# ilia-glushchenko/SimplePathTracer

Hardware: AMD Instinct MI355X
Metric: Msamples/s (pixels×spp/s), RTIOW random-sphere scene, 1/2/4/8 MI355X (higher is better)
Workload: dtype f32

## Files before the change

### simplepathtracer_amd/csrc/spt_device.h

```cpp
#pragma once
#include <hip/hip_runtime.h>
#include <stdint.h>

#include "spt_powf.h"

#pragma clang fp contract(off)

namespace spt {

constexpr uint32_t SPT_SKYBOX_ID = 0, SPT_REFLECTIVE_ID = 1, SPT_REFRACTIVE_ID = 2, SPT_DIFFUSE_ID = 3;

struct f3 {
    float x, y, z;
};

__device__ __forceinline__ f3 mk(float x, float y, float z) { return f3{x, y, z}; }
__device__ __forceinline__ f3 add(f3 a, f3 b) { return f3{a.x + b.x, a.y + b.y, a.z + b.z}; }
__device__ __forceinline__ f3 sub(f3 a, f3 b) { return f3{a.x - b.x, a.y - b.y, a.z - b.z}; }
__device__ __forceinline__ f3 mul(f3 a, float s) { return f3{a.x * s, a.y * s, a.z * s}; }
__device__ __forceinline__ f3 neg(f3 a) { return f3{-a.x, -a.y, -a.z}; }
__device__ __forceinline__ float dot(f3 a, f3 b) { return (a.x * b.x + a.y * b.y) + a.z * b.z; }
__device__ __forceinline__ float lensq(f3 a) { return (a.x * a.x + a.y * a.y) + a.z * a.z; }
__device__ __forceinline__ float sqrt_pos_normal(float h)
{
    float s = __builtin_amdgcn_sqrtf(h);
    const float dn = __builtin_bit_cast(float, __builtin_bit_cast(int, s) - 1);
    const float up = __builtin_bit_cast(float, __builtin_bit_cast(int, s) + 1);
    const float rdn = __builtin_fmaf(-dn, s, h);
    const float rup = __builtin_fmaf(-up, s, h);
    s = rdn <= 0.0f ? dn : s;
    s = rup > 0.0f ? up : s;
    return s;
}

struct Recip {
    float b, rc;
};
__device__ __forceinline__ Recip recip(float b)
{
    float rc = __builtin_amdgcn_rcpf(b);
    const float e = __builtin_fmaf(-b, rc, 1.0f);
    rc = __builtin_fmaf(e, rc, rc);
    return Recip{b, rc};
}
__device__ __forceinline__ float div_core(float a, Recip r)
{
    float q = a * r.rc;
    float e = __builtin_fmaf(-r.b, q, a);
    q = __builtin_fmaf(e, r.rc, q);
    e = __builtin_fmaf(-r.b, q, a);
    return __builtin_fmaf(e, r.rc, q);
}
__device__ __forceinline__ bool div_operand_ok(float x)
{
    const float ax = __builtin_fabsf(x);
    return ax >= 0x1p-40f && ax <= 0x1p40f;
}
__device__ __forceinline__ float div_rn(float a, float b)
{
    float q = div_core(a, recip(b));
    if (__builtin_expect(!(div_operand_ok(a) && div_operand_ok(b)), 0)) q = a / b;
    return q;
}

__device__ __forceinline__ f3 normalize(f3 a)
{
    const float L = lensq(a);
    const Recip r = recip(sqrt_pos_normal(L));
    f3 out = f3{div_core(a.x, r), div_core(a.y, r), div_core(a.z, r)};
    if (__builtin_expect(!(div_operand_ok(a.x) && div_operand_ok(a.y) && div_operand_ok(a.z)), 0)) {
        const float l = __builtin_sqrtf(L);
        out = f3{a.x / l, a.y / l, a.z / l};
    }
    return out;
}
__device__ __forceinline__ f3 reflect(f3 v, f3 n) { return sub(v, mul(mul(n, dot(v, n)), 2.0f)); }

constexpr uint64_t kGamma = 0x9E3779B97F4A7C15ull;

__device__ __forceinline__ uint64_t fmix64(uint64_t z)
{
    z = (z ^ (z >> 30)) * 0xBF58476D1CE4E5B9ull;
    z = (z ^ (z >> 27)) * 0x94D049BB133111EBull;
    return z ^ (z >> 31);
}

__device__ __forceinline__ uint32_t next_u32(uint64_t &st)
{
    st += kGamma;
    uint64_t z = st;
    z = (z ^ (z >> 30)) * 0xBF58476D1CE4E5B9ull;
    z = (z ^ (z >> 27)) * 0x94D049BB133111EBull;
    return (uint32_t)((z ^ (z >> 31)) >> 31);
}

__device__ __forceinline__ float canon_u32(uint32_t bits)
{
    float u = (float)bits * 2.3283064365386963e-10f;
    return u >= 1.0f ? 0x1.fffffep-1f : u;
}
__device__ __forceinline__ float uniform_bits(uint32_t bits, float a, float b)
{
    const float f = __builtin_fminf((float)bits, 0x1.fffffep+31f);
    return __builtin_fmaf(f, 0x1p-32f * (b - a), a);
}
__device__ __forceinline__ float uniform(uint64_t &st, float a, float b) { return uniform_bits(next_u32(st), a, b); }


__device__ __forceinline__ float pow5f(float x) { return spt_glibc_powf(x, 5.f); }

__device__ __forceinline__ float schlick(float rsq, float c) { return rsq + (1.f - rsq) * pow5f(1.f - c); }

__device__ __forceinline__ float refract_k(float r, float c) { return r * c - __builtin_sqrtf(1.f - r * r * (1.f - c * c)); }
__device__ __forceinline__ f3 refract_dir(f3 d, f3 n, float r, float c)
{
    return normalize(add(mul(d, r), mul(n, refract_k(r, c))));
}

__device__ __forceinline__ bool no_tir(float r, float c) { return r * __builtin_sqrtf(1.f - c * c) < 1.f; }

__device__ __forceinline__ uint8_t f2u8(float v)
{
    if (!(v > -2147483648.0f && v < 2147483648.0f)) return 0;
    return (uint8_t)(int32_t)v;
}
__device__ __forceinline__ uint8_t gamma_byte(float c)
{
    return f2u8(__builtin_roundf(__builtin_sqrtf(c / 255.f) * 255.f));
}

}
```

### simplepathtracer_amd/csrc/spt_internal.h

```cpp
#pragma once
#include <hip/hip_runtime.h>
#include <stdint.h>

#include "spt_hip.h"
#include "spt_codes.h"

namespace spt {

struct RowMap {
    uint32_t y0, y1, strip, parts, part;
    uint32_t x0, width;
};

__host__ __device__ inline uint32_t row_of(const RowMap &m, uint32_t lr)
{
    uint32_t blk = lr / m.strip;
    return m.y0 + (blk * m.parts + m.part) * m.strip + (lr - blk * m.strip);
}

__host__ __device__ inline uint32_t rows_owned(const RowMap &m)
{
    if (m.y1 <= m.y0) return 0;
    uint32_t h = m.y1 - m.y0;
    uint32_t period = m.strip * m.parts;
    uint32_t full = h / period, rem = h % period;
    uint32_t r = full * m.strip;
    uint32_t start = m.part * m.strip;
    if (rem > start) r += (rem - start < m.strip) ? rem - start : m.strip;
    return r;
}

__host__ __device__ inline void tile_pixel(uint32_t q, uint32_t width, uint32_t rows, uint32_t &lr, uint32_t &col)
{
    const uint32_t band = (q / width) >> 3;
    const uint32_t h = rows - (band << 3) < 8u ? rows - (band << 3) : 8u;
    const uint32_t qb = q - band * 8u * width;
    const uint32_t ft = width >> 3, wr = width & 7u;
    uint32_t row, c;
    if (h == 8u) {
        const uint32_t t = qb >> 6;
        if (t < ft) {
            row = (qb >> 3) & 7u;
            c = (t << 3) | (qb & 7u);
        } else {
            const uint32_t e = qb - (ft << 6);
            row = e / wr;
            c = (ft << 3) + (e - row * wr);
        }
    } else {
        const uint32_t th = h << 3;
        const uint32_t t = qb / th;
        if (t < ft) {
            const uint32_t e = qb - t * th;
            row = e >> 3;
            c = (t << 3) | (e & 7u);
        } else {
            const uint32_t e = qb - ft * th;
            row = e / wr;
            c = (ft << 3) + (e - row * wr);
        }
    }
    lr = (band << 3) + row;
    col = c;
}


__host__ __device__ inline uint32_t row_of_fast(const RowMap &m, uint32_t lr, const FastDiv &div_strip)
{
    const uint32_t blk = fast_div(lr, div_strip);
    return m.y0 + (blk * m.parts + m.part) * m.strip + (lr - blk * m.strip);
}

struct DealRule {
    uint64_t below;
    uint32_t q, rem;
};
constexpr DealRule make_deal_rule(uint32_t np)
{
    DealRule r{0ull, 0u, 0u};
    if (np == 0u || np > 64u) return r;
    r.q = 64u / np;
    r.rem = 64u - r.q * np;
    uint32_t start = 0;
    for (uint32_t k = 0; k < np; ++k) {
        if (start > 0u) r.below |= 1ull << (start - 1u);
        start += r.q + (k < r.rem ? 1u : 0u);
    }
    return r;
}
struct DealTable {
    DealRule e[65];
    constexpr DealTable() : e{}
    {
        for (uint32_t np = 0; np <= 64u; ++np) e[np] = make_deal_rule(np);
    }
};
static constexpr DealTable kDealTable{};
__host__ __device__ inline uint32_t deal_start(const DealRule &r, uint32_t rank)
{
    return rank * r.q + (rank < r.rem ? rank : r.rem);
}
__host__ __device__ inline uint32_t deal_count(const DealRule &r, uint32_t rank)
{
    return r.q + (rank < r.rem ? 1u : 0u);
}
__host__ __device__ inline void deal_lane(const DealRule &r, uint32_t lane, uint32_t &rank, uint32_t &tt)
{
#ifdef __HIP_DEVICE_COMPILE__
    rank = __builtin_amdgcn_mbcnt_hi((uint32_t)(r.below >> 32), __builtin_amdgcn_mbcnt_lo((uint32_t)r.below, 0u));
#else
    rank = (uint32_t)__builtin_popcountll(r.below & ((1ull << lane) - 1ull));
#endif
    tt = lane - deal_start(r, rank);
}

__host__ __device__ inline void ts_item(uint32_t q, uint32_t width, uint32_t rows, uint32_t S, const FastDiv &div_band,
                                        const FastDiv &div_tile, uint32_t &sl, uint32_t &lr, uint32_t &col)
{
    const uint32_t band = rows >= 8u ? fast_div(q, div_band) : 0u;
    const uint32_t h = rows - (band << 3) < 8u ? rows - (band << 3) : 8u;
    const uint32_t qb = q - band * 8u * width * S;
    const uint32_t ft = width >> 3, wr = width & 7u;
    const uint32_t ti = h * 8u * S;
    uint32_t e, wt, c0;
    if (h == 8u) {
        const uint32_t t = fast_div(qb, div_tile);
        if (t < ft) {
            e = qb - t * 64u * S;
            sl = e >> 6;
            const uint32_t pix = e & 63u;
            lr = (band << 3) + (pix >> 3);
            col = (t << 3) + (pix & 7u);
            return;
        }
        e = qb - ft * ti;
        wt = wr;
        c0 = ft << 3;
    } else {
        const uint32_t t = qb / ti;
        wt = t < ft ? 8u : wr;
        e = qb - (t < ft ? t : ft) * ti;
        c0 = (t < ft ? t : ft) << 3;
    }
    sl = e / (h * wt);
    const uint32_t pix = e - sl * h * wt;
    const uint32_t row = pix / wt;
    lr = (band << 3) + row;
    col = c0 + (pix - row * wt);
}

__host__ __device__ inline void ts_slot_base(uint32_t lr, uint32_t col, uint32_t width, uint32_t rows, uint32_t S,
                                             uint32_t &q0, uint32_t &step)
{
    const uint32_t band = lr >> 3;
    const uint32_t h = rows - (band << 3) < 8u ? rows - (band << 3) : 8u;
    const uint32_t ft = width >> 3, wr = width & 7u;
    const uint32_t t = col >> 3;
    const uint32_t tc = t < ft ? t : ft;
    const uint32_t wt = t < ft ? 8u : wr;
    q0 = band * 8u * width * S + tc * h * 8u * S + (lr - (band << 3)) * wt + (col - (tc << 3));
    step = h * wt;
}


constexpr uint32_t kMaxGroup = 16;
constexpr uint32_t kClusterSlots = 8;
constexpr uint32_t kFlatLeafSlots = 4;
constexpr double kFlatScale = 1.0 - 1e-4;
constexpr double kBoxS = 1.63e-3;
constexpr float kBoxMinDir = 0x1p-20f;
constexpr uint32_t kNoSlot = 0xFFFFFFFFu;
constexpr uint32_t kMiss = 0xFFFFFFFFu;

struct AccelView {
    const float4 *slots;
    const uint32_t *orig;
    const void *nodes;
    uint32_t always_groups, n_nodes;
    uint32_t tree;
    uint32_t leaf_slots;
    const float *kpre;
    float pre_cm;
};

struct PrimLists {
    const uint2 *b8, *b4;
    const uint32_t *slots;
    uint32_t bw;
    uint32_t on;
};
constexpr uint32_t kPrimWalk = 0xFFFFFFFFu;

struct DeviceScene {
    const float4 *shade;
    const uint32_t *mat;
    uint32_t n;
    uint32_t code_stride, code_jmax;
    AccelView accel;
};

struct Camera {
    float view[12];
    float eye[3];
    float sky[3];
};

struct BatchRect {
    uint32_t item_off, item_end, slot_off, pix_off;
    uint32_t x0, y0, w, rows;
    uint32_t npix, alias;
    uint8_t *rgb8;
    FastDiv div_band, div_tile;
};
static_assert(sizeof(BatchRect) == 72, "BatchRect layout");
constexpr uint32_t kInlineRects = 4;

struct RenderArgs {
    DeviceScene scene;
    Camera cam;
    uint32_t width, height, bounces, mode;
    uint64_t seed_key;
    RowMap map;
    uint32_t npix;
    uint32_t spp_batch;
    uint32_t s0;
    uint32_t n_items;
    uint32_t claim;
    FastDiv div_band, div_tile;
    FastDiv div_strip;
    uint32_t *samples;
    uint32_t slot_words;
    uint32_t *head;
    unsigned long long *counters;
    const BatchRect *rects;
    uint32_t n_rects;
    uint32_t n_queues, queue_items;
    uint32_t inline_rects;
    BatchRect rects_inline[kInlineRects];
    uint32_t *svc_ctl;
    const struct SvcJob *svc_jobs;
    const uint32_t *svc_job_claim;
    uint32_t *svc_done;
    unsigned long long *svc_trace;
    uint32_t *svc_host;
    const struct SvcJob *svc_host_jobs;
    const uint32_t *svc_host_job_claim;
    PrimLists prim;
};

constexpr uint32_t kMaxQueues = 8, kQueueStride = 64;
// ... 198 lines not shown
```

### simplepathtracer_amd/csrc/spt_path.h

```cpp
#pragma once
#include "spt_device.h"
#include "spt_internal.h"

#include <float.h>

#ifndef SPT_GROUP
#define SPT_GROUP 4
#endif

#ifndef SPT_DIAG
#define SPT_DIAG 0
#endif
#ifndef SPT_LEAF_SPLIT
#define SPT_LEAF_SPLIT 1
#endif
#ifndef SPT_DUP
#define SPT_DUP 0
#endif
#ifndef SPT_SAMPLER_SKIP0
#define SPT_SAMPLER_SKIP0 1
#endif
#ifndef SPT_SAMPLER_EVEN
#define SPT_SAMPLER_EVEN 1
#endif
// ... 637 lines not shown
    const float ds = lensq(sub(o, p));
    bool better = front && ds < h.best;
    if (__builtin_expect(front && ds == h.best && h.idx != kMiss, 0)) better = orig[s] < orig[h.idx];
    h.best = better ? ds : h.best;
    h.idx = better ? s : h.idx;
    h.t = better ? t : h.t;
}

#ifndef SPT_LANE_LEAF_T
#define SPT_LANE_LEAF_T 24
#endif
#ifndef SPT_LANE_GROUP
#define SPT_LANE_GROUP 2
#endif
#ifndef SPT_LANE_STEPS
#define SPT_LANE_STEPS 8
#endif
template <int LEAF, bool BYTES = false>
__device__ __forceinline__ bool lane_cast(const AccelView &ac, const f3 &o, const f3 &d, bool active, CastDiag &dg,
                                          const uint32_t *lnodes, bool fresh, uint32_t budget, Hit &h, uint32_t &i,
                                          uint32_t &leaf, uint32_t &leaf2)
{
    if (fresh) {
        h.idx = kMiss;
        h.best = FLT_MAX;
        h.t = 0.f;
        i = active ? 0u : (BYTES ? ac.n_nodes << 5 : ac.n_nodes);
        leaf = leaf2 = kNoSlot;
    }
    const float dod = dot(o, d);
    cfloat *slots = (cfloat *)ac.slots;
    const float ddev = lensq(d) - 1.0f;
    const bool no_cull = active && !(ddev <= 1e-6f && ddev >= -1e-6f);
    const float oo = lensq(o);
    if (SPT_DIAG) dg.live_now = (uint32_t)__popcll(__ballot(active));
    for (uint32_t g = 0; g < ac.always_groups; ++g) {
        float4 g4[SPT_GROUP];
#pragma unroll
        for (int k = 0; k < SPT_GROUP; ++k) g4[k] = ld_uniform(slots, g * SPT_GROUP + k);
        test_group<SPT_GROUP>(g4, ac.orig, g * SPT_GROUP, o, d, dod, h, dg);
    }
    auto rcp_dir = [](float x) {
        const float m = __builtin_fmaxf(__builtin_fabsf(x), kBoxMinDir);
        return __builtin_amdgcn_rcpf(__builtin_copysignf(m, x));
    };
    const bool nocull = no_cull || (active && !(oo <= 1e30f));
    float irx, iry, irz, qlx, qly, qlz, qhx, qhy, qhz, neta, kn, sbl;
    auto near_bound = [&](float best) { return __builtin_fmaf(__builtin_amdgcn_sqrtf(best), 1.00001f, kn); };
    auto walk_terms = [&]() {
        const float olen = __builtin_amdgcn_sqrtf(lensq(o)) * 1.000001f;
        const float el = __builtin_fmaf((float)kBoxS, olen, 1e-6f);
        irx = rcp_dir(d.x);
        iry = rcp_dir(d.y);
        irz = rcp_dir(d.z);
        qlx = (-o.x - el) * irx;
        qly = (-o.y - el) * iry;
        qlz = (-o.z - el) * irz;
        qhx = (el - o.x) * irx;
        qhy = (el - o.y) * iry;
        qhz = (el - o.z) * irz;
        const float obs = olen + ac.pre_cm;
        neta = -__builtin_fmaf(1e-6f, obs, 1e-6f);
        kn = __builtin_fmaf(1e-5f, obs, 1e-6f);
        sbl = near_bound(h.best);
    };
    walk_terms();
    const uint4 *ln = (const uint4 *)lnodes;
    const float4 *__restrict__ gs = ac.slots;
    const uint32_t n = BYTES ? ac.n_nodes << 5 : ac.n_nodes;
    uint32_t it = 0;
    for (;;) {
        if (++it > budget) break;
        const bool tr = i < n && leaf2 == kNoSlot;
        const unsigned long long mt = __ballot(tr);
        const unsigned long long mp = __ballot(leaf != kNoSlot);
        if ((mt | mp) == 0ull) break;
        if (mp != 0ull && (mt == 0ull || __popcll(mp) >= SPT_LANE_LEAF_T)) {
            if (SPT_DIAG) {
                const unsigned long long nl = (unsigned long long)__popcll(mp);
                dg.leaves += 1;
                dg.pairs += nl;
                dg.lane_tests += (unsigned long long)LEAF * nl;
            }
            if (leaf != kNoSlot) {
#pragma unroll 1
                for (int k0 = 0; k0 < LEAF; k0 += SPT_LANE_GROUP) {
                    float4 m[SPT_LANE_GROUP];
#pragma unroll
                    for (int k = 0; k < SPT_LANE_GROUP; ++k) m[k] = gs[leaf + k0 + k];
#pragma unroll
                    for (int k = 0; k < SPT_LANE_GROUP; ++k) {
                        float tc, hh;
                        if (ray_sphere(m[k], o, d, tc, hh))
                            update_member_lane(tc, hh, ac.orig, leaf + k0 + k, o, d, dod, h);
                    }
                }
                sbl = near_bound(h.best);
                leaf = leaf2;
                leaf2 = kNoSlot;
            }
            continue;
        }
        if (SPT_DIAG) dg.live += 1;
        auto visit = [&]() {
            const uint4 *rec = BYTES ? (const uint4 *)((const char *)lnodes + i) : ln + 2 * i;
            const uint4 ra = rec[0], rb = rec[1];
            const uint32_t nskip = rb.x, nslot = rb.y;
            const float ax = __builtin_fmaf(__uint_as_float(ra.x), irx, qlx);
            const float bx = __builtin_fmaf(__uint_as_float(ra.w), irx, qhx);
            const float ay = __builtin_fmaf(__uint_as_float(ra.y), iry, qly);
            const float by = __builtin_fmaf(__uint_as_float(rb.z), iry, qhy);
            const float az = __builtin_fmaf(__uint_as_float(ra.z), irz, qlz);
            const float bz = __builtin_fmaf(__uint_as_float(rb.w), irz, qhz);
            const float tn = max3_raw(__builtin_fminf(ax, bx), __builtin_fminf(ay, by),
                                      max_raw(__builtin_fminf(az, bz), neta));
            const float tf = min3_raw(__builtin_fmaxf(ax, bx), __builtin_fmaxf(ay, by),
                                      min_raw(__builtin_fmaxf(az, bz), sbl));
            const bool hit = (tn <= tf) | nocull;
            const bool is_leaf = nslot != kNoSlot;
            if (hit && is_leaf) {
                leaf2 = leaf;
                leaf = nslot;
            }
            i = (hit && !is_leaf) ? i + (BYTES ? 32u : 1u) : nskip;
        };
#pragma unroll
        for (int k = 0; k < SPT_LANE_STEPS; ++k) {
            const bool w = i < n && leaf2 == kNoSlot;
            if (SPT_DIAG) dg.nodes += (unsigned long long)__popcll(__ballot(w));
            if (w) visit();
        }
    }
    return !(i < n || leaf != kNoSlot);
}

template <int LEAF>
__device__ __forceinline__ Hit find_closest_lane(const AccelView &ac, const f3 &o, const f3 &d, bool active,
                                                 CastDiag &dg, const uint32_t *lnodes)
{
    Hit h;
    uint32_t i, leaf, leaf2;
    (void)lane_cast<LEAF>(ac, o, d, active, dg, lnodes, true, 0xFFFFFFFFu, h, i, leaf, leaf2);
    return h;
}

struct Path {
    uint32_t phase, item, bounce, spec;
    uint64_t st;
    f3 o, d;
    uint32_t slot;
    uint32_t job;
};

__device__ __forceinline__ f3 coop_ball_vector(uint64_t &st, bool need, uint32_t *lds, unsigned long long *rounds = nullptr)
{
    const uint32_t lane = __lane_id();
    const uint64_t st0 = st;
    f3 r;
    uint32_t jacc = 0;
    unsigned long long pend;
    uint32_t jb;
    const unsigned long long needm = __ballot(need);
    if (SPT_SAMPLER_SKIP0 && __popcll(needm) <= 32) {
        r = mk(0.f, 0.f, 0.f);
        pend = needm;
        jb = 0;
    } else {
        uint64_t t = st0;
        r.x = uniform(t, -0.5f, 0.5f);
        r.y = uniform(t, -0.5f, 0.5f);
        r.z = uniform(t, -0.5f, 0.5f);
        pend = __ballot(need && lensq(r) < 0.25f);
        jb = 1;
    }
    const uint32_t s_lo = (uint32_t)st0, s_hi = (uint32_t)(st0 >> 32);
    if (SPT_DIAG && rounds) rounds[0] += 1;
#if SPT_DIAG
    const unsigned long long t_in = __builtin_amdgcn_s_memtime();
#endif
#if SPT_SAMPLER_EVEN
    if (jb != 0u) jacc = __builtin_amdgcn_inverse_ballot_w64(pend) ? 1u : 0u;
    while (pend != 0ull) {
        if (SPT_DIAG && rounds) rounds[1] += 1;
        const DealRule dr = kDealTable.e[__popcll(pend)];
        const bool is_p = __builtin_amdgcn_inverse_ballot_w64(pend);
        const uint32_t rank = lane_rank(pend);
        if (is_p) lds[rank] = (jacc << 6) | lane;
        uint32_t pidx, tt;
        deal_lane(dr, lane, pidx, tt);
        const uint32_t w = lds[pidx];
        const uint32_t src = w & 63u;
        const uint32_t h_lo = (uint32_t)__shfl((int)s_lo, (int)src), h_hi = (uint32_t)__shfl((int)s_hi, (int)src);
        uint64_t b = (((uint64_t)h_hi << 32) | h_lo) + (uint64_t)(3u * ((w >> 6) + tt)) * kGamma;
        f3 c;
        c.x = uniform(b, -0.5f, 0.5f);
        c.y = uniform(b, -0.5f, 0.5f);
        c.z = uniform(b, -0.5f, 0.5f);
        const unsigned long long acc = __ballot(!(lensq(c) < 0.25f));
        const uint32_t start = deal_start(dr, rank), cnt = deal_count(dr, rank);
        const unsigned long long seg = acc >> (start & 63u);
        const uint32_t tstar = seg != 0ull ? (uint32_t)__builtin_ctzll(seg) : 64u;
        const bool found = is_p && tstar < cnt;
        const uint32_t from = found ? start + tstar : lane;
        const float rx = __shfl(c.x, (int)from), ry = __shfl(c.y, (int)from), rz = __shfl(c.z, (int)from);
        if (found) r = mk(rx, ry, rz);
        if (is_p) jacc += tstar < cnt ? tstar : cnt;
        pend = __ballot(is_p && !found);
    }
#else
    while (pend != 0ull) {
        if (SPT_DIAG && rounds) rounds[1] += 1;
        const uint32_t np = (uint32_t)__popcll(pend);
        uint32_t lg = np <= 4u ? 4u : (uint32_t)__builtin_clz(np - 1u) - 26u;
        lg = lg > 4u ? 4u : lg;
        const bool is_p = __builtin_amdgcn_inverse_ballot_w64(pend);
        const uint32_t rank = lane_rank(pend);
        if (is_p) lds[rank] = lane;
        const uint32_t pidx = lane >> lg, tt = lane & ((1u << lg) - 1u);
        const bool valid = pidx < np;
        const uint32_t src = lds[valid ? pidx : 0u];
        const uint32_t h_lo = (uint32_t)__shfl((int)s_lo, (int)src), h_hi = (uint32_t)__shfl((int)s_hi, (int)src);
        uint64_t b = (((uint64_t)h_hi << 32) | h_lo) + (uint64_t)(3u * (jb + tt)) * kGamma;
        f3 c;
        c.x = uniform(b, -0.5f, 0.5f);
        c.y = uniform(b, -0.5f, 0.5f);
        c.z = uniform(b, -0.5f, 0.5f);
        const unsigned long long acc = __ballot(valid && !(lensq(c) < 0.25f));
        const uint32_t seg = is_p ? (uint32_t)(acc >> (rank << lg)) & ((1u << (1u << lg)) - 1u) : 0u;
        const bool found = seg != 0u;
        const uint32_t tstar = found ? (uint32_t)__builtin_ctz(seg) : 0u;
        const uint32_t from = found ? (rank << lg) + tstar : lane;
        const float rx = __shfl(c.x, (int)from), ry = __shfl(c.y, (int)from), rz = __shfl(c.z, (int)from);
        if (found) {
            r = mk(rx, ry, rz);
            jacc = jb + tstar;
        }
        pend = __ballot(is_p && !found);
        jb += 1u << lg;
    }
#endif
    if (need) st = st0 + (uint64_t)(3u * (jacc + 1u)) * kGamma;
#if SPT_DIAG
    if (rounds) rounds[2] += __builtin_amdgcn_s_memtime() - t_in;
#endif
    return r;
}

typedef __attribute__((address_space(4))) const RenderArgs kargs_t;
__device__ __forceinline__ kargs_t *kernarg_args()
{
    uint32_t z;
    asm volatile("s_mov_b32 %0, 0" : "=s"(z));
    typedef __attribute__((address_space(4))) const char kchar;
    return (kargs_t *)((kchar *)__builtin_amdgcn_kernarg_segment_ptr() + z);
}

__device__ __forceinline__ bool prim_list_cast(const AccelView &ac, const f3 &o, const f3 &d, bool active, uint32_t pxy,
                                               Hit &h, CastDiag &dg)
{
    kargs_t &k = *kernarg_args();
    const float ddev = lensq(d) - 1.0f;
    if (__ballot(active && !(ddev <= 1e-6f && ddev >= -1e-6f && lensq(o) <= 1e30f)) != 0ull) return false;
    h.idx = kMiss;
    h.best = FLT_MAX;
    h.t = 0.f;
    const unsigned long long live = __ballot(active);
    if (live == 0ull) return true;
    const uint32_t bw = k.prim.bw;
    const uint32_t x = pxy & 0xFFFFu, y = pxy >> 16;
    const float dod = dot(o, d);
    cfloat *slots = (cfloat *)ac.slots;
    cuint *ids = (cuint *)k.prim.slots;
    if (SPT_DIAG) dg.live_now = (uint32_t)__popcll(live);
    auto test_run = [&](uint2 e) {
        for (uint32_t i = e.x; i < e.x + e.y; i += 4u) {
            uint32_t s[4];
            float4 sp[4];
#pragma unroll
            for (int q = 0; q < 4; ++q) s[q] = ids[i + q];
#pragma unroll
            for (int q = 0; q < 4; ++q) sp[q] = ld_uniform(slots, s[q]);
            float tcv[4], hv[4];
            bool pass[4];
#pragma unroll
            for (int q = 0; q < 4; ++q) pass[q] = ray_sphere(sp[q], o, d, tcv[q], hv[q]);
            if (SPT_DIAG) dg.lane_tests += 4ull * dg.live_now;
#pragma unroll
            for (int q = 0; q < 4; ++q) {
                const unsigned long long pm = __ballot(pass[q]);
                if (SPT_DIAG) {
                    dg.spheres += 1;
                    dg.branches += pm != 0ull ? 1 : 0;
                }
                if (pm != 0ull) update_member(pm, tcv[q], hv[q], ac.orig, s[q], o, d, dod, h, dg);
            }
        }
    };
    const uint32_t b8 = (y >> 3) * bw + (x >> 3);
    const uint32_t lead = __builtin_amdgcn_readlane(b8, (int)__builtin_ctzll(live));
    if (__ballot(active && b8 != lead) == 0ull) {
        cuint *blk = (cuint *)k.prim.b8 + 2u * lead;
        const uint2 e = make_uint2(blk[0], blk[1]);
        if (e.y == kPrimWalk) return false;
        test_run(e);
        return true;
    }
    const uint32_t b4 = (y >> 2) * bw + (x >> 3);
    unsigned long long todo = live;
    while (todo != 0ull) {
        const uint32_t b = __builtin_amdgcn_readlane(b4, (int)__builtin_ctzll(todo));
        cuint *blk = (cuint *)k.prim.b4 + 2u * b;
        const uint2 e = make_uint2(blk[0], blk[1]);
        if (e.y == kPrimWalk) return false;
        test_run(e);
        todo &= ~__ballot(active && b4 == b);
    }
    return true;
}

__device__ __forceinline__ void refract_event(const float4 *__restrict__ slots, Path &ps, uint32_t idx)
{
    const float4 cs = slots[idx];
    const f3 C = mk(cs.x, cs.y, cs.z);
    const f3 nrm = normalize(sub(ps.o, C));
    const f3 d = ps.d;
    const float cc = dot(neg(nrm), d);
    f3 nd;
    if (uniform(ps.st, 0.f, 1.f) < schlick(kRsq, cc)) {
        nd = reflect(d, nrm);
    } else if (no_tir(kAirToGlass, cc)) {
        const f3 d2 = refract_dir(d, nrm, kAirToGlass, cc);
        const f3 rs = sub(C, ps.o);
        const float tc = dot(rs, d2);
        const float dd = lensq(rs) - tc * tc;
        const float t = tc + __builtin_sqrtf(cs.w - dd);
        ps.o = mk(ps.o.x + d2.x * t, ps.o.y + d2.y * t, ps.o.z + d2.z * t);
        const f3 n2 = neg(normalize(sub(ps.o, C)));
        const float c2 = dot(neg(n2), d2);
        if (uniform(ps.st, 0.f, 1.f) < schlick(kRsq, c2))
            nd = reflect(d2, n2);
        else if (no_tir(kGlassToAir, c2))
            nd = refract_dir(d2, n2, kGlassToAir, c2);
        else
            nd = reflect(d2, n2);
    } else {
        nd = reflect(d, nrm);
    }
    ps.d = nd;
}

template <bool WT = false>
__device__ __forceinline__ void finish_step(uint32_t mode, uint32_t *samples, Path &ps, bool fin, bool spec_event,
                                            bool refr_event, bool sky, uint32_t word, unsigned long long &done,
                                            unsigned long long &dropped)
{
    bool counted = true;
    if (spec_event) {
        const uint32_t k = ps.spec & 0xFFFFu;
        if (mode == 1u && k < kTaskPasses && refr_event) ps.spec |= 1u << (16u + k);
        ++ps.spec;
        if (mode == 1u && k + 1u >= kTaskPasses) {
            fin = true;
            counted = false;
            word = kZeroWord;
            ++dropped;
        } else if (k + 1u > kSpecularCap) {
            fin = true;
            word = kZeroWord;
        }
    }
    if (fin) {
        typedef __attribute__((address_space(1))) uint32_t gu32_t;
        typedef __attribute__((address_space(1))) unsigned long long gu64_t;
        if (mode == 0u) {
            if (WT)
                __hip_atomic_store((gu32_t *)(samples + ps.item), word, __ATOMIC_RELAXED, __HIP_MEMORY_SCOPE_AGENT);
            else
                samples[ps.item] = word;
        } else {
            const uint32_t key =
                counted ? 1u + (((ps.spec & 0xFFFFu) << 11) | (sky ? 1u << 10 : 0u) | ((ps.spec >> 16) & 0x3FFu)) : 0u;
            if (WT)
                __hip_atomic_store((gu64_t *)(samples + (size_t)2 * ps.item), (unsigned long long)word | ((unsigned long long)key << 32),
                                   __ATOMIC_RELAXED, __HIP_MEMORY_SCOPE_AGENT);
            else
                *(uint2 *)(samples + (size_t)2 * ps.item) = make_uint2(word, key);
        }
        ps.phase = PH_IDLE;
        ps.d = mk(0.f, 0.f, 0.f);
        ++done;
    }
}

template <bool KARG, bool WT, bool SAMPLER>
__device__ __forceinline__ void shade_step_body(const RenderArgs &a, Path &ps, const Hit &h, bool act,
                                                unsigned long long &done, unsigned long long &dropped, uint32_t *lds,
                                                unsigned long long *diag_rounds)
{
    const float4 *__restrict__ hit = a.scene.accel.slots;
    const float4 *__restrict__ shade = a.scene.shade;
    const uint32_t *__restrict__ mat = a.scene.mat;
    uint32_t *samples = a.samples;
    uint32_t mode = a.mode;
    uint32_t bounces = a.bounces, code_stride = a.scene.code_stride, code_jmax = a.scene.code_jmax;
    if constexpr (KARG) {
        kargs_t &k = *kernarg_args();
        hit = k.scene.accel.slots;
        shade = k.scene.shade;
        mat = k.scene.mat;
        samples = k.samples;
        mode = k.mode;
        bounces = k.bounces;
        code_stride = k.scene.code_stride;
        code_jmax = k.scene.code_jmax;
    }
    const uint32_t idx = h.idx;
    bool fin = false;
    uint32_t word = kZeroWord;
    const bool dl = ps.phase == PH_DLOOP;
    uint32_t m = SPT_SKYBOX_ID;
    if (act && idx != kMiss) m = mat[idx];
    bool scatter = false, refr = false;
    if (!act) {
    } else if (dl) {
        --ps.bounce;
        const bool end = ps.bounce == 0u || idx == kMiss;
        if (end) {
            const uint32_t j = min(bounces - ps.bounce - 1u, code_jmax);
            word = code_word(diffuse_code(j, ps.slot, code_stride));
            fin = true;
        }
        scatter = !end;
        refr = false;
    } else {
        scatter = m == SPT_DIFFUSE_ID || m == SPT_REFLECTIVE_ID;
        refr = m == SPT_REFRACTIVE_ID;
        if (!scatter && !refr) {
            word = __float_as_uint(ps.d.y + 1.f);
            fin = true;
        }
    }
    bool spec_event = false;
    const f3 rv_coop = SAMPLER ? coop_ball_vector(ps.st, scatter, lds, diag_rounds) : opaque_v3(mk(0.1f, 0.2f, 0.3f));
    if ((SPT_DUP & 2) && SAMPLER) {
        uint64_t st2 = opaque_v(ps.st);
        const f3 r2 = coop_ball_vector(st2, opaque_v(scatter ? 1u : 0u) != 0u, lds);
        sink_v(r2.x);
        sink_v(r2.y);
        sink_v(r2.z);
        sink_v(st2);
    }
    if (scatter) {
        const float4 cs = hit[idx];
        const f3 C = mk(cs.x, cs.y, cs.z);
        ps.o = contact(ps.o, ps.d, h.t);
        const f3 nrm = normalize(sub(ps.o, C));
        f3 rv = rv_coop;
        f3 base;
        if (dl) {
            base = add(ps.o, nrm);
        } else if (m == SPT_DIFFUSE_ID) {
            ps.slot = idx;
            base = nrm;
            ps.phase = PH_DLOOP;
        } else {
            base = reflect(ps.d, nrm);
            rv = mul(rv, shade[idx].w);
            spec_event = true;
        }
        ps.d = normalize(add(base, rv));
    }
    if (refr) {
        ps.o = contact(ps.o, ps.d, h.t);
        if (SPT_DUP & 256) {
            Path p2 = ps;
            p2.o = opaque_v3(p2.o);
            refract_event(hit, p2, idx);
            sink_v(p2.d.x);
            sink_v(p2.o.x);
            sink_v(p2.st);
        }
        refract_event(hit, ps, idx);
        spec_event = true;
    }
    finish_step<WT>(mode, samples, ps, fin, spec_event, refr, !dl, word, done, dropped);
}
template <bool KARG = false, bool WT = false>
__device__ __forceinline__ void shade_step(const RenderArgs &a, Path &ps, const Hit &h, bool act,
                                           unsigned long long &done, unsigned long long &dropped, uint32_t *lds,
                                           unsigned long long *diag_rounds = nullptr)
{
    if (SPT_DUP & 128) {
        Path p2 = ps;
        p2.o = opaque_v3(p2.o);
        p2.d = opaque_v3(p2.d);
        Hit h2 = h;
        h2.t = opaque_v(h2.t);
        unsigned long long d2 = 0, x2 = 0;
        shade_step_body<KARG, WT, false>(a, p2, h2, act, d2, x2, lds, nullptr);
        sink_v(p2.o.x);
        sink_v(p2.d.x);
        sink_v(p2.st);
    }
    shade_step_body<KARG, WT, true>(a, ps, h, act, done, dropped, lds, diag_rounds);
}



__device__ __forceinline__ void start_path(const RenderArgs &a, uint32_t mine, uint32_t rows, const Recip &rw,
                                           const Recip &rh, const f3 &eye, Path &ps, uint32_t *pxy = nullptr)
{
    uint32_t sl, lr, cx;
    ts_item(mine, a.map.width, rows, a.spp_batch, a.div_band, a.div_tile, sl, lr, cx);
    const uint32_t s = a.s0 + sl;
    ps.item = mine;
    const uint32_t x = a.map.x0 + cx;
    const uint32_t y = a.map.parts == 1u ? a.map.y0 + lr : row_of_fast(a.map, lr, a.div_strip);
    if (pxy) *pxy = (y << 16) | x;
    ps.st = fmix64(a.seed_key ^ (((uint64_t)(y * a.width + x) << 32) | (uint64_t)s));
    const float un = (float)y + uniform(ps.st, -1.f, 1.f);
    const float vn = (float)x + uniform(ps.st, -1.f, 1.f);
    float u = div_core(un, rw), v = div_core(vn, rh);
    if (__builtin_expect(!(div_operand_ok(un) && div_operand_ok(vn)), 0)) {
        u = un / (float)a.width;
        v = vn / (float)a.height;
    }
    const float vx = -1.f + 2.f * v, vy = -1.f + 2.f * u;
    const float *m = a.cam.view;
    ps.d = normalize(mk((m[0] * vx + m[1] * vy) + (m[2] * 1.f + m[3] * 0.f),
                        (m[4] * vx + m[5] * vy) + (m[6] * 1.f + m[7] * 0.f),
                        (m[8] * vx + m[9] * vy) + (m[10] * 1.f + m[11] * 0.f)));
    ps.o = eye;
    ps.phase = PH_TRACE;
    ps.bounce = a.bounces;
    ps.spec = 0;
}

__device__ __forceinline__ void start_path_kernarg(uint32_t mine, uint32_t rows, Path &ps, uint32_t *pxy = nullptr)
{
    kargs_t &k = *kernarg_args();
    RenderArgs a;
    a.map = RowMap{k.map.y0, k.map.y1, k.map.strip, k.map.parts, k.map.part, k.map.x0, k.map.width};
    a.width = k.width;
    a.height = k.height;
    a.bounces = k.bounces;
    a.npix = k.npix;
    a.n_items = k.n_items;
    a.spp_batch = k.spp_batch;
    a.s0 = k.s0;
    a.seed_key = k.seed_key;
    a.div_band = FastDiv{k.div_band.d, k.div_band.m, k.div_band.s};
    a.div_tile = FastDiv{k.div_tile.d, k.div_tile.m, k.div_tile.s};
    a.div_strip = FastDiv{k.div_strip.d, k.div_strip.m, k.div_strip.s};
#pragma unroll
    for (int q = 0; q < 12; ++q) a.cam.view[q] = k.cam.view[q];
    start_path(a, mine, rows, recip((float)a.width), recip((float)a.height),
               mk(k.cam.eye[0], k.cam.eye[1], k.cam.eye[2]), ps, pxy);
}

typedef __attribute__((address_space(4))) const BatchRect crect_t;
__device__ __forceinline__ uint32_t find_rect(uint32_t nb)
{
    kargs_t &k = *kernarg_args();
    crect_t *r = k.inline_rects ? (crect_t *)k.rects_inline : (crect_t *)k.rects;
    uint32_t lo = 0, hi = k.n_rects;
    while (hi - lo > 1u) {
        const uint32_t mid = (lo + hi) >> 1;
        if (r[mid].item_off <= nb) lo = mid; else hi = mid;
    }
    return lo;
}

__device__ __forceinline__ void start_path_rect(uint32_t mine, uint32_t ri, Path &ps, uint32_t *pxy = nullptr)
{
    kargs_t &k = *kernarg_args();
    crect_t &r = (k.inline_rects ? (crect_t *)k.rects_inline : (crect_t *)k.rects)[ri];
    if (mine >= r.item_end) return;
    RenderArgs a;
    a.map = RowMap{r.y0, r.y0 + r.rows, 1u, 1u, 0u, r.x0, r.w};
    a.width = k.width;
    a.height = k.height;
    a.bounces = k.bounces;
    a.npix = r.npix;
    a.spp_batch = k.spp_batch;
    a.s0 = k.s0;
    a.seed_key = k.seed_key;
    a.div_band = FastDiv{r.div_band.d, r.div_band.m, r.div_band.s};
    a.div_tile = FastDiv{r.div_tile.d, r.div_tile.m, r.div_tile.s};
    a.div_strip = FastDiv{1u, 0u, 0u};
#pragma unroll
    for (int q = 0; q < 12; ++q) a.cam.view[q] = k.cam.view[q];
    start_path(a, mine - r.item_off, r.rows, recip((float)a.width), recip((float)a.height),
               mk(k.cam.eye[0], k.cam.eye[1], k.cam.eye[2]), ps, pxy);
    ps.item += r.slot_off;
}

__device__ __forceinline__ void start_path_svc(uint32_t mine, const uint32_t *rec, Path &ps, uint32_t *pxy = nullptr)
{
    auto f = [&](int i) -> uint32_t { return (uint32_t)__builtin_amdgcn_readfirstlane(rec[i]); };
    if (mine >= f(1)) return;
    kargs_t &k = *kernarg_args();
    RenderArgs a;
    a.map = RowMap{f(8), f(9), f(10), f(11), f(12), f(13), f(14)};
    a.width = k.width;
    a.height = k.height;
    a.bounces = k.bounces;
    a.spp_batch = f(5);
    a.s0 = f(6);
    a.seed_key = k.seed_key;
    a.div_band = FastDiv{f(15), f(16), f(17)};
    a.div_tile = FastDiv{f(18), f(19), f(20)};
    a.div_strip = FastDiv{f(21), f(22), f(23)};
#pragma unroll
    for (int q = 0; q < 12; ++q) a.cam.view[q] = k.cam.view[q];
    start_path(a, mine - f(0), f(4), recip((float)a.width), recip((float)a.height),
               mk(k.cam.eye[0], k.cam.eye[1], k.cam.eye[2]), ps, pxy);
    ps.item += f(2);
    ps.job = f(3);
}

}
}
```

Baseline: 25710.

## Convert shade step control flow to wave-uniform ballot masks

Rewrites the shading step so material classification, termination and scatter decisions are held as 64-bit wave ballot masks (SGPRs) rather than per-lane booleans. Lane predicates are recovered with inverse_ballot, and normalize's slow-path check uses min3/max3 plus a ballot. The sampler loads its deal table as 16-byte scalar loads from constant memory, and finish_step gets a specialized early path for mode 0. The aim is to cut VALU compare and exec-mask bookkeeping and divergent branching in the hot shading loop, at the cost of inline asm and heavier reliance on compiler handling of the ballot intrinsics.

```diff
diff --git a/simplepathtracer_amd/csrc/spt_device.h b/simplepathtracer_amd/csrc/spt_device.h
--- a/simplepathtracer_amd/csrc/spt_device.h
+++ b/simplepathtracer_amd/csrc/spt_device.h
@@ -63,14 +63,25 @@
     return q;
 }
 
+__device__ __forceinline__ unsigned long long normalize_slow_mask(f3 a, float L)
+{
+    float lo, hi;
+    asm("v_min3_f32 %0, |%1|, |%2|, |%3|" : "=v"(lo) : "v"(a.x), "v"(a.y), "v"(a.z));
+    asm("v_max3_f32 %0, |%1|, |%2|, |%3|" : "=v"(hi) : "v"(a.x), "v"(a.y), "v"(a.z));
+    return __ballot(!(lo >= 0x1p-40f)) | __ballot(!(hi <= 0x1p40f)) | __ballot(!(L <= 0x1p82f));
+}
 __device__ __forceinline__ f3 normalize(f3 a)
 {
     const float L = lensq(a);
     const Recip r = recip(sqrt_pos_normal(L));
     f3 out = f3{div_core(a.x, r), div_core(a.y, r), div_core(a.z, r)};
-    if (__builtin_expect(!(div_operand_ok(a.x) && div_operand_ok(a.y) && div_operand_ok(a.z)), 0)) {
+    const unsigned long long slow = normalize_slow_mask(a, L);
+    if (__builtin_expect(slow != 0ull, 0)) {
+        const bool mine = __builtin_amdgcn_inverse_ballot_w64(slow);
         const float l = __builtin_sqrtf(L);
-        out = f3{a.x / l, a.y / l, a.z / l};
+        out.x = mine ? a.x / l : out.x;
+        out.y = mine ? a.y / l : out.y;
+        out.z = mine ? a.z / l : out.z;
     }
     return out;
 }
diff --git a/simplepathtracer_amd/csrc/spt_internal.h b/simplepathtracer_amd/csrc/spt_internal.h
--- a/simplepathtracer_amd/csrc/spt_internal.h
+++ b/simplepathtracer_amd/csrc/spt_internal.h
@@ -95,7 +95,7 @@
         for (uint32_t np = 0; np <= 64u; ++np) e[np] = make_deal_rule(np);
     }
 };
-static constexpr DealTable kDealTable{};
+alignas(16) static constexpr DealTable kDealTable{};
 __host__ __device__ inline uint32_t deal_start(const DealRule &r, uint32_t rank)
 {
     return rank * r.q + (rank < r.rem ? rank : r.rem);
diff --git a/simplepathtracer_amd/csrc/spt_path.h b/simplepathtracer_amd/csrc/spt_path.h
--- a/simplepathtracer_amd/csrc/spt_path.h
+++ b/simplepathtracer_amd/csrc/spt_path.h
@@ -813,7 +813,7 @@
     uint32_t job;
 };
 
-__device__ __forceinline__ f3 coop_ball_vector(uint64_t &st, bool need, uint32_t *lds, unsigned long long *rounds = nullptr)
+__device__ __forceinline__ f3 coop_ball_vector(uint64_t &st, unsigned long long needm, uint32_t *lds, unsigned long long *rounds = nullptr)
 {
     const uint32_t lane = __lane_id();
     const uint64_t st0 = st;
@@ -821,7 +821,6 @@
     uint32_t jacc = 0;
     unsigned long long pend;
     uint32_t jb;
-    const unsigned long long needm = __ballot(need);
     if (SPT_SAMPLER_SKIP0 && __popcll(needm) <= 32) {
         r = mk(0.f, 0.f, 0.f);
         pend = needm;
@@ -831,7 +830,7 @@
         r.x = uniform(t, -0.5f, 0.5f);
         r.y = uniform(t, -0.5f, 0.5f);
         r.z = uniform(t, -0.5f, 0.5f);
-        pend = __ballot(need && lensq(r) < 0.25f);
+        pend = needm & __ballot(lensq(r) < 0.25f);
         jb = 1;
     }
     const uint32_t s_lo = (uint32_t)st0, s_hi = (uint32_t)(st0 >> 32);
@@ -841,9 +840,14 @@
 #endif
 #if SPT_SAMPLER_EVEN
     if (jb != 0u) jacc = __builtin_amdgcn_inverse_ballot_w64(pend) ? 1u : 0u;
+    typedef uint32_t u32x4 __attribute__((ext_vector_type(4)));
+    typedef __attribute__((address_space(4))) const u32x4 cu32x4;
+    cu32x4 *deal = (cu32x4 *)&kDealTable.e[0];
+    asm volatile("" : "+s"(deal));
     while (pend != 0ull) {
         if (SPT_DIAG && rounds) rounds[1] += 1;
-        const DealRule dr = kDealTable.e[__popcll(pend)];
+        const u32x4 dw = deal[__popcll(pend)];
+        const DealRule dr{((uint64_t)dw.y << 32) | dw.x, dw.z, dw.w};
         const bool is_p = __builtin_amdgcn_inverse_ballot_w64(pend);
         const uint32_t rank = lane_rank(pend);
         if (is_p) lds[rank] = (jacc << 6) | lane;
@@ -861,12 +865,13 @@
         const uint32_t start = deal_start(dr, rank), cnt = deal_count(dr, rank);
         const unsigned long long seg = acc >> (start & 63u);
         const uint32_t tstar = seg != 0ull ? (uint32_t)__builtin_ctzll(seg) : 64u;
-        const bool found = is_p && tstar < cnt;
+        const unsigned long long foundm = pend & __ballot(tstar < cnt);
+        const bool found = __builtin_amdgcn_inverse_ballot_w64(foundm);
         const uint32_t from = found ? start + tstar : lane;
         const float rx = __shfl(c.x, (int)from), ry = __shfl(c.y, (int)from), rz = __shfl(c.z, (int)from);
         if (found) r = mk(rx, ry, rz);
         if (is_p) jacc += tstar < cnt ? tstar : cnt;
-        pend = __ballot(is_p && !found);
+        pend &= ~foundm;
     }
 #else
     while (pend != 0ull) {
@@ -900,7 +905,7 @@
         jb += 1u << lg;
     }
 #endif
-    if (need) st = st0 + (uint64_t)(3u * (jacc + 1u)) * kGamma;
+    if (__builtin_amdgcn_inverse_ballot_w64(needm)) st = st0 + (uint64_t)(3u * (jacc + 1u)) * kGamma;
 #if SPT_DIAG
     if (rounds) rounds[2] += __builtin_amdgcn_s_memtime() - t_in;
 #endif
@@ -1011,13 +1016,33 @@
 }
 
 template <bool WT = false>
-__device__ __forceinline__ void finish_step(uint32_t mode, uint32_t *samples, Path &ps, bool fin, bool spec_event,
-                                            bool refr_event, bool sky, uint32_t word, unsigned long long &done,
-                                            unsigned long long &dropped)
-{
+__device__ __forceinline__ void finish_step(uint32_t mode, uint32_t *samples, Path &ps, unsigned long long finm,
+                                            unsigned long long specm, unsigned long long refrm, unsigned long long skym,
+                                            uint32_t word, unsigned long long &done, unsigned long long &dropped)
+{
+    typedef __attribute__((address_space(1))) uint32_t gu32_t;
+    typedef __attribute__((address_space(1))) unsigned long long gu64_t;
+    const uint32_t k = ps.spec & 0xFFFFu;
+    const bool spec_event = __builtin_amdgcn_inverse_ballot_w64(specm);
+    if (mode == 0u) {
+        ps.spec += spec_event ? 1u : 0u;
+        const unsigned long long capm = specm & __ballot(k + 1u > kSpecularCap);
+        word = __builtin_amdgcn_inverse_ballot_w64(capm) ? kZeroWord : word;
+        if (__builtin_amdgcn_inverse_ballot_w64(finm | capm)) {
+            if (WT)
+                __hip_atomic_store((gu32_t *)(samples + ps.item), word, __ATOMIC_RELAXED, __HIP_MEMORY_SCOPE_AGENT);
+            else
+                samples[ps.item] = word;
+            ps.phase = PH_IDLE;
+            ps.d = mk(0.f, 0.f, 0.f);
+            ++done;
+        }
+        return;
+    }
+    bool fin = __builtin_amdgcn_inverse_ballot_w64(finm);
+    const bool refr_event = __builtin_amdgcn_inverse_ballot_w64(refrm), sky = __builtin_amdgcn_inverse_ballot_w64(skym);
     bool counted = true;
     if (spec_event) {
-        const uint32_t k = ps.spec & 0xFFFFu;
         if (mode == 1u && k < kTaskPasses && refr_event) ps.spec |= 1u << (16u + k);
         ++ps.spec;
         if (mode == 1u && k + 1u >= kTaskPasses) {
@@ -1031,22 +1056,13 @@
         }
     }
     if (fin) {
-        typedef __attribute__((address_space(1))) uint32_t gu32_t;
-        typedef __attribute__((address_space(1))) unsigned long long gu64_t;
-        if (mode == 0u) {
-            if (WT)
-                __hip_atomic_store((gu32_t *)(samples + ps.item), word, __ATOMIC_RELAXED, __HIP_MEMORY_SCOPE_AGENT);
-            else
-                samples[ps.item] = word;
-        } else {
-            const uint32_t key =
-                counted ? 1u + (((ps.spec & 0xFFFFu) << 11) | (sky ? 1u << 10 : 0u) | ((ps.spec >> 16) & 0x3FFu)) : 0u;
-            if (WT)
-                __hip_atomic_store((gu64_t *)(samples + (size_t)2 * ps.item), (unsigned long long)word | ((unsigned long long)key << 32),
-                                   __ATOMIC_RELAXED, __HIP_MEMORY_SCOPE_AGENT);
-            else
-                *(uint2 *)(samples + (size_t)2 * ps.item) = make_uint2(word, key);
-        }
+        const uint32_t key =
+            counted ? 1u + (((ps.spec & 0xFFFFu) << 11) | (sky ? 1u << 10 : 0u) | ((ps.spec >> 16) & 0x3FFu)) : 0u;
+        if (WT)
+            __hip_atomic_store((gu64_t *)(samples + (size_t)2 * ps.item), (unsigned long long)word | ((unsigned long long)key << 32),
+                               __ATOMIC_RELAXED, __HIP_MEMORY_SCOPE_AGENT);
+        else
+            *(uint2 *)(samples + (size_t)2 * ps.item) = make_uint2(word, key);
         ps.phase = PH_IDLE;
         ps.d = mk(0.f, 0.f, 0.f);
         ++done;
@@ -1076,62 +1092,53 @@
         code_jmax = k.scene.code_jmax;
     }
     const uint32_t idx = h.idx;
-    bool fin = false;
+    const unsigned long long actm = __ballot(act);
+    const unsigned long long hitm = actm & __ballot(idx != kMiss);
+    uint32_t m = SPT_SKYBOX_ID;
+    if (__builtin_amdgcn_inverse_ballot_w64(hitm)) m = mat[idx];
+    const unsigned long long dlm = actm & __ballot(ps.phase == PH_DLOOP);
+    const bool dl = __builtin_amdgcn_inverse_ballot_w64(dlm);
+    const uint32_t nb = ps.bounce - 1u;
+    ps.bounce = dl ? nb : ps.bounce;
+    const unsigned long long endm = dlm & (__ballot(nb == 0u) | ~hitm);
+    const unsigned long long trm = actm & ~dlm;
+    const unsigned long long diffm = trm & __ballot(m == SPT_DIFFUSE_ID);
+    const unsigned long long mirm = trm & __ballot(m == SPT_REFLECTIVE_ID);
+    const unsigned long long refrm = trm & __ballot(m == SPT_REFRACTIVE_ID);
+    const unsigned long long skym = trm & ~(diffm | mirm | refrm);
+    const unsigned long long scatm = (dlm & ~endm) | diffm | mirm;
+    const uint32_t j = min(bounces - nb - 1u, code_jmax);
     uint32_t word = kZeroWord;
-    const bool dl = ps.phase == PH_DLOOP;
-    uint32_t m = SPT_SKYBOX_ID;
-    if (act && idx != kMiss) m = mat[idx];
-    bool scatter = false, refr = false;
-    if (!act) {
-    } else if (dl) {
-        --ps.bounce;
-        const bool end = ps.bounce == 0u || idx == kMiss;
-        if (end) {
-            const uint32_t j = min(bounces - ps.bounce - 1u, code_jmax);
-            word = code_word(diffuse_code(j, ps.slot, code_stride));
-            fin = true;
-        }
-        scatter = !end;
-        refr = false;
-    } else {
-        scatter = m == SPT_DIFFUSE_ID || m == SPT_REFLECTIVE_ID;
-        refr = m == SPT_REFRACTIVE_ID;
-        if (!scatter && !refr) {
-            word = __float_as_uint(ps.d.y + 1.f);
-            fin = true;
-        }
-    }
-    bool spec_event = false;
-    const f3 rv_coop = SAMPLER ? coop_ball_vector(ps.st, scatter, lds, diag_rounds) : opaque_v3(mk(0.1f, 0.2f, 0.3f));
+    word = __builtin_amdgcn_inverse_ballot_w64(endm) ? code_word(diffuse_code(j, ps.slot, code_stride)) : word;
+    word = __builtin_amdgcn_inverse_ballot_w64(skym) ? __float_as_uint(ps.d.y + 1.f) : word;
+    const f3 rv_coop = SAMPLER ? coop_ball_vector(ps.st, scatm, lds, diag_rounds) : opaque_v3(mk(0.1f, 0.2f, 0.3f));
     if ((SPT_DUP & 2) && SAMPLER) {
         uint64_t st2 = opaque_v(ps.st);
-        const f3 r2 = coop_ball_vector(st2, opaque_v(scatter ? 1u : 0u) != 0u, lds);
+        const bool scatter = __builtin_amdgcn_inverse_ballot_w64(scatm);
+        const f3 r2 = coop_ball_vector(st2, __ballot(opaque_v(scatter ? 1u : 0u) != 0u), lds);
         sink_v(r2.x);
         sink_v(r2.y);
         sink_v(r2.z);
         sink_v(st2);
     }
-    if (scatter) {
+    if (__builtin_amdgcn_inverse_ballot_w64(scatm)) {
         const float4 cs = hit[idx];
         const f3 C = mk(cs.x, cs.y, cs.z);
         ps.o = contact(ps.o, ps.d, h.t);
         const f3 nrm = normalize(sub(ps.o, C));
         f3 rv = rv_coop;
-        f3 base;
-        if (dl) {
-            base = add(ps.o, nrm);
-        } else if (m == SPT_DIFFUSE_ID) {
-            ps.slot = idx;
-            base = nrm;
-            ps.phase = PH_DLOOP;
-        } else {
+        const f3 on = add(ps.o, nrm);
+        f3 base = mk(dl ? on.x : nrm.x, dl ? on.y : nrm.y, dl ? on.z : nrm.z);
+        if (__builtin_amdgcn_inverse_ballot_w64(mirm)) {
             base = reflect(ps.d, nrm);
             rv = mul(rv, shade[idx].w);
-            spec_event = true;
         }
         ps.d = normalize(add(base, rv));
     }
-    if (refr) {
+    const bool first = __builtin_amdgcn_inverse_ballot_w64(diffm);
+    ps.slot = first ? idx : ps.slot;
+    ps.phase = first ? PH_DLOOP : ps.phase;
+    if (__builtin_amdgcn_inverse_ballot_w64(refrm)) {
         ps.o = contact(ps.o, ps.d, h.t);
         if (SPT_DUP & 256) {
             Path p2 = ps;
@@ -1142,9 +1149,8 @@
             sink_v(p2.st);
         }
         refract_event(hit, ps, idx);
-        spec_event = true;
-    }
-    finish_step<WT>(mode, samples, ps, fin, spec_event, refr, !dl, word, done, dropped);
+    }
+    finish_step<WT>(mode, samples, ps, endm | skym, mirm | refrm, refrm, trm, word, done, dropped);
 }
 template <bool KARG = false, bool WT = false>
 __device__ __forceinline__ void shade_step(const RenderArgs &a, Path &ps, const Hit &h, bool act,
```

Measured after the change: 26290 (median of 6 runs). 2.3% higher.
